# MoayedHajiAli/ElasticDiffusion-official

Hardware: AMD Instinct MI355X
Metric: images/sec at 50 steps (SDXL 2048x1024) (higher is better)
Workload: dtype fp16

## Files before the change

elasticdiffusion_official_amd/csrc/attention_kernels.hip:

```cpp
#include <hip/hip_runtime.h>
#include <stdint.h>

#include "elastic_hip.h"

namespace {

constexpr int D = 64;
constexpr int QB = 128;
constexpr int KT = 64;
constexpr int K_LD = 72;
constexpr int V_LD_TR = 96;
constexpr int V_LD_T = 68;

typedef float f32x16 __attribute__((ext_vector_type(16)));
typedef float f32x8 __attribute__((ext_vector_type(8)));
typedef short s16x4 __attribute__((ext_vector_type(4)));
typedef short s16x8 __attribute__((ext_vector_type(8)));
typedef __bf16 bf16x8 __attribute__((ext_vector_type(8)));
typedef _Float16 f16x8 __attribute__((ext_vector_type(8)));

struct alignas(16) Vec16 { uint32_t w[4]; };
struct alignas(8) Vec8 { uint32_t w[2]; };

struct BF {
  typedef bf16x8 v8;
  static __device__ __forceinline__ f32x16 mfma(v8 a, v8 b, f32x16 c) {
    return __builtin_amdgcn_mfma_f32_32x32x16_bf16(a, b, c, 0, 0, 0);
  }
  static __device__ __forceinline__ v8 pack(f32x8 p) { return __builtin_convertvector(p, v8); }
};
struct HF {
  typedef f16x8 v8;
  static __device__ __forceinline__ f32x16 mfma(v8 a, v8 b, f32x16 c) {
    return __builtin_amdgcn_mfma_f32_32x32x16_f16(a, b, c, 0, 0, 0);
  }
  static __device__ __forceinline__ v8 pack(f32x8 p) { return __builtin_convertvector(p, v8); }
};

template <typename V8>
__device__ __forceinline__ V8 as_v8(Vec16 x) {
  return __builtin_bit_cast(V8, x);
}

struct Params {
  const uint16_t* q;
  const uint16_t* k;
  const uint16_t* v;
  uint16_t* o;
  int Nq, Nk, H, BH, nqb;
  int64_t q_sb, q_sn, k_sb, k_sn, v_sb, v_sn, o_sb, o_sn;
  float scale_log2e;
};

template <bool TR>
// ... 174 lines not shown
          const int row = 16 * st + 4 * hi + ((lane & 15) >> 2);
          const int col = 32 * db + 16 * ((lane >> 4) & 1) + 4 * (lane & 3);
          typedef s16x4 __attribute__((address_space(3))) * lds_s16x4_ptr;
          const s16x4 lo = __builtin_amdgcn_ds_read_tr16_b64_v4i16((lds_s16x4_ptr)(&sm.v[buf][row * V_LD_TR + col]));
          const s16x4 hi4 = __builtin_amdgcn_ds_read_tr16_b64_v4i16((lds_s16x4_ptr)(&sm.v[buf][(row + 8) * V_LD_TR + col]));
          const s16x8 both = __builtin_shufflevector(lo, hi4, 0, 1, 2, 3, 4, 5, 6, 7);
          vf = __builtin_bit_cast(Vec16, both);
        } else {
          const uint16_t* vrow = &sm.v[buf][(32 * db + ln) * V_LD_T + 16 * st + 4 * hi];
          const Vec8 lo = *reinterpret_cast<const Vec8*>(vrow);
          const Vec8 hi8 = *reinterpret_cast<const Vec8*>(vrow + 8);
          vf.w[0] = lo.w[0], vf.w[1] = lo.w[1], vf.w[2] = hi8.w[0], vf.w[3] = hi8.w[1];
        }
#pragma unroll
        for (int qn = 0; qn < QN; ++qn) oacc[qn][db] = T::mfma(as_v8<typename T::v8>(vf), pf[qn], oacc[qn][db]);
      }
    }

    if (t + 1 < n_tiles) write_lds(buf ^ 1);
    __syncthreads();
  }

#pragma unroll
  for (int qn = 0; qn < QN; ++qn) {
    const float l_tot = l_run[qn] + __shfl_xor(l_run[qn], 32, 64);
    const float inv = 1.0f / l_tot;
    if (q_row[qn] < p.Nq) {
      uint16_t* orow = og + (int64_t)q_row[qn] * p.o_sn;
#pragma unroll
      for (int db = 0; db < 2; ++db)
#pragma unroll
        for (int g = 0; g < 4; ++g) {
          f32x8 tmp;
#pragma unroll
          for (int e = 0; e < 4; ++e) tmp[e] = oacc[qn][db][4 * g + e] * inv, tmp[4 + e] = 0.f;
          const Vec16 packed = __builtin_bit_cast(Vec16, T::pack(tmp));
          Vec8 out8 = {{packed.w[0], packed.w[1]}};
          *reinterpret_cast<Vec8*>(orow + 32 * db + 8 * g + 4 * hi) = out8;
        }
    }
  }
}


constexpr float RESCALE_LOG2 = 6.0f;
constexpr float RESCALE_SUM_MAX = 64.0f;

template <int NK>
struct SmemPipe {
  uint16_t k[NK][KT * K_LD];
  uint16_t v[3][KT * V_LD_TR];
};

template <typename T>
__device__ __forceinline__ void qk_tile(const uint16_t* kt, int ln, int hi, const typename T::v8 (&qf)[4], f32x16 (&s)[2]) {
#pragma unroll
  for (int i = 0; i < 16; ++i) s[0][i] = s[1][i] = 0.f;
#pragma unroll
  for (int ks = 0; ks < 4; ++ks)
#pragma unroll
    for (int kb = 0; kb < 2; ++kb) {
      const Vec16 kf = *reinterpret_cast<const Vec16*>(&kt[(32 * kb + ln) * K_LD + 16 * ks + 8 * hi]);
      s[kb] = T::mfma(as_v8<typename T::v8>(kf), qf[ks], s[kb]);
    }
}

__device__ __forceinline__ Vec16 v_frag_tr(const uint16_t* vt, int lane, int hi, int st, int db) {
  const int row = 16 * st + 4 * hi + ((lane & 15) >> 2);
  const int col = 32 * db + 16 * ((lane >> 4) & 1) + 4 * (lane & 3);
  typedef s16x4 __attribute__((address_space(3))) * lds_s16x4_ptr;
  const s16x4 lo = __builtin_amdgcn_ds_read_tr16_b64_v4i16((lds_s16x4_ptr)(&vt[row * V_LD_TR + col]));
  const s16x4 hi4 = __builtin_amdgcn_ds_read_tr16_b64_v4i16((lds_s16x4_ptr)(&vt[(row + 8) * V_LD_TR + col]));
  return __builtin_bit_cast(Vec16, __builtin_shufflevector(lo, hi4, 0, 1, 2, 3, 4, 5, 6, 7));
}

template <typename T>
__device__ __forceinline__ void pv_tile(const uint16_t* vt, int lane, int hi, const typename T::v8 (&pf)[4], f32x16 (&o)[2]) {
#pragma unroll
  for (int st = 0; st < 4; ++st)
#pragma unroll
    for (int db = 0; db < 2; ++db)
      o[db] = T::mfma(as_v8<typename T::v8>(v_frag_tr(vt, lane, hi, st, db)), pf[st], o[db]);
}

typedef __amdgpu_buffer_rsrc_t BufRsrc;
typedef uint32_t u32x4 __attribute__((ext_vector_type(4)));
__device__ __forceinline__ BufRsrc make_rsrc(const void* base, int64_t bytes) {
  const uint64_t a = (uint64_t)base;
  const uint32_t lo = __builtin_amdgcn_readfirstlane((int)(uint32_t)a), hi = __builtin_amdgcn_readfirstlane((int)(uint32_t)(a >> 32));
  const uint32_t n = __builtin_amdgcn_readfirstlane((int)(uint32_t)(bytes > 0xffffffffll ? 0xffffffffll : (bytes < 0 ? 0 : bytes)));
  return __builtin_amdgcn_make_buffer_rsrc((void*)(((uint64_t)hi << 32) | lo),  0, (int)n, 0x00020000);
}
__device__ __forceinline__ Vec16 buf_load16(BufRsrc rs, uint32_t voff, uint32_t soff) {
  const u32x4 v = __builtin_bit_cast(u32x4, __builtin_amdgcn_raw_buffer_load_b128(rs, voff, soff, 0));
  Vec16 o = {{v[0], v[1], v[2], v[3]}};
  return o;
}


template <typename T, int NDB = 2>
__device__ __forceinline__ void store_o_row(uint16_t* orow, const f32x16 (&o)[NDB], float inv, int hi, bool valid, int dh = 64) {
#pragma unroll
  for (int db = 0; db < NDB; ++db) {
    uint32_t part[4][2];
#pragma unroll
    for (int g = 0; g < 4; ++g) {
      f32x8 tmp;
#pragma unroll
      for (int e = 0; e < 4; ++e) tmp[e] = o[db][4 * g + e] * inv, tmp[4 + e] = 0.f;
      const Vec16 packed = __builtin_bit_cast(Vec16, T::pack(tmp));
      part[g][0] = packed.w[0], part[g][1] = packed.w[1];
    }
#pragma unroll
    for (int gp = 0; gp < 2; ++gp) {
      const int ge = 2 * gp, go = 2 * gp + 1;
      const uint32_t r0 = __shfl_xor(hi ? part[ge][0] : part[go][0], 32, 64);
      const uint32_t r1 = __shfl_xor(hi ? part[ge][1] : part[go][1], 32, 64);
      Vec16 out;
      if (hi) out = Vec16{{r0, r1, part[go][0], part[go][1]}};
      else out = Vec16{{part[ge][0], part[ge][1], r0, r1}};
      const int d0 = 32 * db + 8 * (hi ? go : ge);
      if (valid && d0 < dh) *reinterpret_cast<Vec16*>(orow + d0) = out;
    }
  }
}

struct True { static constexpr bool value = true; };
struct False { static constexpr bool value = false; };

struct SoftmaxRun {
  float mb;
  float l;
  float mx;
  float use;
  float alpha;
  float psum;
};

template <typename T>
__device__ __forceinline__ void softmax_slice(int i, f32x16 (&s)[2], float sl, SoftmaxRun& r, typename T::v8 (&pf)[4]) {
  if (i < 2) {
    float mx = (i == 0) ? -INFINITY : r.mx;
#pragma unroll
    for (int j = 0; j < 16; j += 2) mx = fmaxf(fmaxf(mx, s[i][j]), s[i][j + 1]);
    r.mx = mx;
    asm volatile("" : "+v"(r.mx));
  } else if (i == 2) {
    const float mx = fmaxf(r.mx, __shfl_xor(r.mx, 32, 64));
    const float mbn = mx * sl;
    r.use = (mbn - r.mb > RESCALE_LOG2) ? mbn : r.mb;
    r.alpha = __builtin_amdgcn_exp2f(r.mb - r.use);
    r.mb = r.use;
    r.psum = 0.f;
    asm volatile("" : "+v"(r.use), "+v"(r.alpha));
  } else if (i < 15) {
    const int g = (i - 3) / 3, w = (i - 3) % 3;
    const int f0 = 8 * g + 3 * w, n = (w == 2) ? 2 : 3;
#pragma unroll
    for (int j = 0; j < n; ++j) {
      const int f = f0 + j;
      const float e = __builtin_amdgcn_exp2f(__builtin_fmaf(s[f >> 4][f & 15], sl, -r.use));
      s[f >> 4][f & 15] = e;
      r.psum += e;
    }
    asm volatile("" : "+v"(r.psum));
    if (w == 2) {
      f32x8 pv;
#pragma unroll
      for (int j = 0; j < 8; ++j) pv[j] = s[g >> 1][8 * (g & 1) + j];
      pf[g] = T::pack(pv);
      asm volatile("" : "+v"(pf[g]));
    }
  } else {
    r.l = __builtin_fmaf(r.l, r.alpha, r.psum);
  }
}

template <typename T, bool EXP2>
__device__ __forceinline__ void softmax_slice_lazy(int i, f32x16 (&s)[2], float sl, SoftmaxRun& r, typename T::v8 (&pf)[4]) {
  if (i == 0) r.psum = 0.f;
#pragma unroll
  for (int j = 0; j < 2; ++j) {
    const int f = 2 * i + j;
    const float e = EXP2 ? __builtin_amdgcn_exp2f(s[f >> 4][f & 15])
                         : __builtin_amdgcn_exp2f(__builtin_fmaf(s[f >> 4][f & 15], sl, -r.mb));
    s[f >> 4][f & 15] = e;
    r.psum += e;
  }
  asm volatile("" : "+v"(r.psum));
  if ((i & 3) == 3) {
    const int g = i >> 2;
    f32x8 pv;
#pragma unroll
    for (int j = 0; j < 8; ++j) pv[j] = s[g >> 1][8 * (g & 1) + j];
    pf[g] = T::pack(pv);
    asm volatile("" : "+v"(pf[g]));
  }
}

template <typename T>
__device__ __forceinline__ void resoftmax_tile(const uint16_t* kt, int ln, int hi, const typename T::v8 (&qf)[4],
                                               f32x16 (&s)[2], float sl, SoftmaxRun& r, typename T::v8 (&pf)[4]) {
  qk_tile<T>(kt, ln, hi, qf, s);
  float mx = s[0][0];
#pragma unroll
  for (int j = 1; j < 16; ++j) mx = fmaxf(mx, s[0][j]);
#pragma unroll
  for (int j = 0; j < 16; ++j) mx = fmaxf(mx, s[1][j]);
  mx = fmaxf(mx, __shfl_xor(mx, 32, 64));
  const float use = fmaxf(r.mb, mx * sl);
  r.alpha = __builtin_amdgcn_exp2f(r.mb - use);
  r.mb = use;
  float psum = 0.f;
#pragma unroll
  for (int g = 0; g < 4; ++g) {
    f32x8 pv;
#pragma unroll
    for (int j = 0; j < 8; ++j) {
      const int f = 8 * g + j;
      pv[j] = __builtin_amdgcn_exp2f(__builtin_fmaf(s[f >> 4][f & 15], sl, -use));
      psum += pv[j];
    }
    pf[g] = T::pack(pv);
  }
  r.psum = psum;
}

template <typename T, bool HAS_PV, bool HAS_NEXT, bool LAZY, bool EXP2, int DEPTH, class Filler>
__device__ __forceinline__ void pipe_region(Filler&& filler, const uint16_t* k_next, const uint16_t* v_prev, int lane, int ln, int hi,
                                            const typename T::v8 (&qf)[4], f32x16 (&s_cur)[2], f32x16 (&s_next)[2],
                                            const typename T::v8 (&p_prev)[4], typename T::v8 (&p_cur)[4],
                                            f32x16 (&o)[2], float sl, SoftmaxRun& run, const f32x16& negm) {
  constexpr int NQK = HAS_NEXT ? 8 : 0, N = NQK + (HAS_PV ? 8 : 0);
  auto fetch = [&](int i) -> Vec16 {
    if (i < NQK) return *reinterpret_cast<const Vec16*>(&k_next[(32 * (i & 1) + ln) * K_LD + 16 * (i >> 1) + 8 * hi]);
    const int j = i - NQK;
    return v_frag_tr(v_prev, lane, hi, j >> 1, j & 1);
  };
  if (HAS_NEXT && !EXP2) {
#pragma unroll
    for (int i = 0; i < 16; ++i) s_next[0][i] = s_next[1][i] = 0.f;
  }
  Vec16 ring[DEPTH + 1];
#pragma unroll
  for (int r = 0; r <= DEPTH; ++r) ring[r] = Vec16{{0u, 0u, 0u, 0u}};
#pragma unroll
  for (int r = 0; r < DEPTH; ++r)
    if (r < N) ring[r] = fetch(r);
#pragma unroll
  for (int i = 0; i < 16; ++i) {
    if (i < N) {
      if (i + DEPTH < N) ring[(i + DEPTH) % (DEPTH + 1)] = fetch(i + DEPTH);
      const Vec16 a_cur = ring[i % (DEPTH + 1)];
      if (i < NQK) {
        if (EXP2 && i < 2) s_next[i & 1] = T::mfma(as_v8<typename T::v8>(a_cur), qf[0], negm);
        else s_next[i & 1] = T::mfma(as_v8<typename T::v8>(a_cur), qf[i >> 1], s_next[i & 1]);
        asm volatile("" : "+v"(s_next[i & 1]));
      } else {
        const int j = i - NQK;
        o[j & 1] = T::mfma(as_v8<typename T::v8>(a_cur), p_prev[j >> 1], o[j & 1]);
        asm volatile("" : "+v"(o[j & 1]));
      }
    }
    if (LAZY) softmax_slice_lazy<T, EXP2>(i, s_cur, sl, run, p_cur);
    else softmax_slice<T>(i, s_cur, sl, run, p_cur);
    filler(i);
    __builtin_amdgcn_sched_barrier(0);
  }
}

template <typename T, bool LAZY, bool EXP2 = false, int DEPTH = 1, int WAVES = 4>
__global__ void __launch_bounds__(64 * WAVES, 2)
k_flash_attn_pipe(const Params p) {
  static_assert(LAZY || !EXP2, "the exponent-domain variant is built on the lazy-maximum loop");
  static_assert(WAVES == 4 || WAVES == 8, "4 or 8 waves per workgroup");
  constexpr int NK = LAZY ? 3 : 2;
  constexpr int NST = 8 / WAVES;
  __shared__ SmemPipe<NK> sm;
  const int tid = threadIdx.x;
  const int lane = tid & 63, wave = tid >> 6;
  const int ln = lane & 31, hi = lane >> 5;
  int bh, qblk;
  {
    const int id = blockIdx.x, per = 8 * p.nqb, grp = id / per, r = id - grp * per;
    if ((grp + 1) * 8 <= p.BH) {
      bh = grp * 8 + (r & 7);
      qblk = r >> 3;
    } else {
      bh = grp * 8 + r / p.nqb;
      qblk = r % p.nqb;
    }
  }
  const int b = bh / p.H, h = bh - b * p.H;
  const uint16_t* qg = p.q + b * p.q_sb + h * D;
  const uint16_t* kg = p.k + b * p.k_sb + h * D;
  const uint16_t* vg = p.v + b * p.v_sb + h * D;
  uint16_t* og = p.o + b * p.o_sb + h * D;

  const int q_row = qblk * (32 * WAVES) + wave * 32 + ln;
  typename T::v8 qf[4];
#pragma unroll
  for (int ks = 0; ks < 4; ++ks) qf[ks] = as_v8<typename T::v8>(load_row16(qg, p.q_sn, q_row, p.Nq, 16 * ks + 8 * hi));

  const BufRsrc k_rs = make_rsrc(kg, ((int64_t)(p.Nk - 1) * p.k_sn + D) * 2);
  const BufRsrc v_rs = make_rsrc(vg, ((int64_t)(p.Nk - 1) * p.v_sn + D) * 2);
  const int st_row = tid >> 3, st_col = (tid & 7) * 8;
  const uint32_t k_off = (uint32_t)(((int64_t)st_row * p.k_sn + st_col) * 2), k_half = (uint32_t)(32 * p.k_sn * 2);
  const uint32_t v_off = (uint32_t)(((int64_t)st_row * p.v_sn + st_col) * 2), v_half = (uint32_t)(32 * p.v_sn * 2);
  Vec16 kreg[NST], vreg[NST];
  auto load_k = [&](int t) {
    const uint32_t base = k_off + (uint32_t)t * 2u * k_half;
#pragma unroll
    for (int i = 0; i < NST; ++i) kreg[i] = buf_load16(k_rs, base + i * k_half, 0);
  };
  auto load_v = [&](int t) {
    const uint32_t base = v_off + (uint32_t)t * 2u * v_half;
#pragma unroll
    for (int i = 0; i < NST; ++i) vreg[i] = buf_load16(v_rs, base + i * v_half, 0);
  };
  auto write_k = [&](int buf) {
#pragma unroll
    for (int i = 0; i < NST; ++i) *reinterpret_cast<Vec16*>(&sm.k[buf][(st_row + 32 * i) * K_LD + st_col]) = kreg[i];
  };
  auto write_v = [&](int buf) {
#pragma unroll
    for (int i = 0; i < NST; ++i) *reinterpret_cast<Vec16*>(&sm.v[buf][(st_row + 32 * i) * V_LD_TR + st_col]) = vreg[i];
  };

  f32x16 oacc[2];
#pragma unroll
  for (int i = 0; i < 16; ++i) oacc[0][i] = oacc[1][i] = 0.f;
  SoftmaxRun run;
  run.mb = -INFINITY, run.l = 0.f, run.mx = 0.f, run.use = 0.f, run.alpha = 1.f, run.psum = 0.f;
  const float sl = EXP2 ? 1.0f : p.scale_log2e;
  const int n_tiles = (p.Nk + KT - 1) / KT, n_full = p.Nk / KT;
  f32x16 negm;
#pragma unroll
  for (int i = 0; i < 16; ++i) negm[i] = 0.f;

  load_k(0);
  load_v(0);
  Vec16 k1reg[NST];
#pragma unroll
  for (int i = 0; i < NST; ++i) k1reg[i] = buf_load16(k_rs, k_off + 2u * k_half + i * k_half, 0);
  write_k(0);
  write_v(0);
#pragma unroll
  for (int i = 0; i < NST; ++i) *reinterpret_cast<Vec16*>(&sm.k[1][(st_row + 32 * i) * K_LD + st_col]) = k1reg[i];
  __syncthreads();

  f32x16 sA[2], sB[2];
  typename T::v8 pA[4], pB[4];
  int vb_prev = 2, vb_cur = 0, vb_next = 1;
  int kb_cur = 0, kb_next = 1, kb_write = NK == 3 ? 2 : 0;

  auto iter = [&](auto has_pv, auto has_next, int t, f32x16 (&s_cur)[2], f32x16 (&s_next)[2],
                  typename T::v8 (&p_prev)[4], typename T::v8 (&p_cur)[4]) {
    const uint32_t kbase = k_off + (uint32_t)(t + 2) * 2u * k_half, vbase = v_off + (uint32_t)(t + 1) * 2u * v_half;
    uint16_t* const kdst = sm.k[kb_write];
    uint16_t* const vdst = sm.v[vb_next];
    auto filler = [&](int i) {
      if (i < NST) kreg[i] = buf_load16(k_rs, kbase + i * k_half, 0);
      else if (i < 2 * NST) vreg[i - NST] = buf_load16(v_rs, vbase + (i - NST) * v_half, 0);
      else if (i >= 11 && i < 11 + NST) *reinterpret_cast<Vec16*>(&kdst[(st_row + 32 * (i - 11)) * K_LD + st_col]) = kreg[i - 11];
      else if (i >= 11 + NST && i < 11 + 2 * NST)
        *reinterpret_cast<Vec16*>(&vdst[(st_row + 32 * (i - 11 - NST)) * V_LD_TR + st_col]) = vreg[i - 11 - NST];
    };
    constexpr bool lazy = LAZY && (EXP2 || decltype(has_pv)::value);
    pipe_region<T, decltype(has_pv)::value, decltype(has_next)::value, lazy, EXP2, DEPTH>(filler, sm.k[kb_next], sm.v[vb_prev], lane, ln,
                                                                                          hi, qf, s_cur, s_next, p_prev, p_cur,
                                                                                          oacc, sl, run, negm);
    if (lazy) {
      run.alpha = 1.0f;
      if (__any(!(run.psum <= RESCALE_SUM_MAX))) {
        const float mb_old = run.mb;
        resoftmax_tile<T>(sm.k[kb_cur], ln, hi, qf, s_cur, sl, run, p_cur);
        if (EXP2) {
          const float d = run.mb - mb_old;
          if (decltype(has_next)::value) {
#pragma unroll
            for (int i = 0; i < 16; ++i) s_next[0][i] -= d, s_next[1][i] -= d;
          }
#pragma unroll
          for (int i = 0; i < 16; ++i) negm[i] = -run.mb;
          asm volatile("" : "+v"(negm));
        }
      }
      run.l = __builtin_fmaf(run.l, run.alpha, run.psum);
    }
    if (__any(run.alpha != 1.0f)) {
#pragma unroll
      for (int i = 0; i < 16; ++i) {
        oacc[0][i] *= run.alpha;
        oacc[1][i] *= run.alpha;
      }
    }
    const int tmp = vb_prev;
    vb_prev = vb_cur, vb_cur = vb_next, vb_next = tmp;
    const int ktmp = kb_cur;
    kb_cur = kb_next, kb_next = kb_write, kb_write = NK == 3 ? ktmp : kb_cur;
    __syncthreads();
  };

  if (n_full > 0) {
    qk_tile<T>(sm.k[0], ln, hi, qf, sA);
    if (EXP2) {
      float mx = sA[0][0];
#pragma unroll
      for (int j = 1; j < 16; ++j) mx = fmaxf(mx, sA[0][j]);
#pragma unroll
      for (int j = 0; j < 16; ++j) mx = fmaxf(mx, sA[1][j]);
      mx = fmaxf(mx, __shfl_xor(mx, 32, 64));
      run.mb = mx;
#pragma unroll
      for (int i = 0; i < 16; ++i) sA[0][i] -= mx, sA[1][i] -= mx, negm[i] = -mx;
      asm volatile("" : "+v"(negm));
    }
    __syncthreads();
    if (n_full == 1) {
      iter(False{}, False{}, 0, sA, sB, pB, pA);
    } else {
      iter(False{}, True{}, 0, sA, sB, pB, pA);
      int t = 1;
      for (; t + 2 < n_full; t += 2) {
        iter(True{}, True{}, t, sB, sA, pA, pB);
        iter(True{}, True{}, t + 1, sA, sB, pB, pA);
      }
      if (n_full - t == 2) {
        iter(True{}, True{}, t, sB, sA, pA, pB);
        iter(True{}, False{}, t + 1, sA, sB, pB, pA);
      } else {
        iter(True{}, False{}, t, sB, sA, pA, pB);
      }
    }
    if ((n_full - 1) & 1) pv_tile<T>(sm.v[vb_prev], lane, hi, pB, oacc);
    else pv_tile<T>(sm.v[vb_prev], lane, hi, pA, oacc);
  }

  if (n_tiles > n_full) {
    f32x16 s[2];
    qk_tile<T>(sm.k[kb_cur], ln, hi, qf, s);
#pragma unroll
    for (int kb = 0; kb < 2; ++kb)
#pragma unroll
      for (int r = 0; r < 16; ++r)
        if (n_full * KT + 32 * kb + 8 * (r >> 2) + 4 * hi + (r & 3) >= p.Nk) s[kb][r] = -INFINITY;
    float mx = s[0][0];
#pragma unroll
    for (int r = 1; r < 16; ++r) mx = fmaxf(mx, s[0][r]);
#pragma unroll
    for (int r = 0; r < 16; ++r) mx = fmaxf(mx, s[1][r]);
    mx = fmaxf(mx, __shfl_xor(mx, 32, 64));
    const float use = fmaxf(run.mb, mx * sl);
    const float alpha = __builtin_amdgcn_exp2f(run.mb - use);
    float psum = 0.f;
#pragma unroll
    for (int kb = 0; kb < 2; ++kb)
#pragma unroll
      for (int r = 0; r < 16; ++r) {
        const float e = __builtin_amdgcn_exp2f(__builtin_fmaf(s[kb][r], sl, -use));
        s[kb][r] = e;
        psum += e;
      }
    run.l = __builtin_fmaf(run.l, alpha, psum);
#pragma unroll
    for (int i = 0; i < 16; ++i) {
      oacc[0][i] *= alpha;
      oacc[1][i] *= alpha;
    }
    typename T::v8 pf[4];
#pragma unroll
    for (int st = 0; st < 4; ++st) {
      f32x8 pv;
#pragma unroll
      for (int j = 0; j < 8; ++j) pv[j] = s[st >> 1][8 * (st & 1) + j];
      pf[st] = T::pack(pv);
    }
    pv_tile<T>(sm.v[vb_cur], lane, hi, pf, oacc);
  }

  const float l_tot = run.l + __shfl_xor(run.l, 32, 64);
  const float inv = 1.0f / l_tot;
  store_o_row<T>(og + (int64_t)q_row * p.o_sn, oacc, inv, hi, q_row < p.Nq);
}

constexpr int SK_QBLOCKS = 4;

template <int NKB>
struct SmemSmall {
  uint16_t k[32 * NKB * K_LD];
  uint16_t v[32 * NKB * V_LD_TR];
};

template <typename T, int NKB>
__global__ void __launch_bounds__(256, 2)
k_flash_attn_smallkv(const Params p) {
  __shared__ SmemSmall<NKB> sm;
  const int tid = threadIdx.x;
  const int lane = tid & 63, wave = tid >> 6;
  const int ln = lane & 31, hi = lane >> 5;
  const int nqg = p.nqb;
  const int bh = blockIdx.x / nqg, qgrp = blockIdx.x - bh * nqg;
  const int b = bh / p.H, h = bh - b * p.H;
  const uint16_t* qg = p.q + b * p.q_sb + h * D;
  const uint16_t* kg = p.k + b * p.k_sb + h * D;
  const uint16_t* vg = p.v + b * p.v_sb + h * D;
  uint16_t* og = p.o + b * p.o_sb + h * D;

  for (int idx = tid; idx < 32 * NKB * 8; idx += 256) {
    const int row = idx >> 3, col = (idx & 7) * 8;
    *reinterpret_cast<Vec16*>(&sm.k[row * K_LD + col]) = load_row16(kg, p.k_sn, row, p.Nk, col);
    *reinterpret_cast<Vec16*>(&sm.v[row * V_LD_TR + col]) = load_row16(vg, p.v_sn, row, p.Nk, col);
  }
  __syncthreads();
  const float sl = p.scale_log2e;

  for (int qb = 0; qb < SK_QBLOCKS; ++qb) {
    const int q_row = (qgrp * SK_QBLOCKS + qb) * QB + wave * 32 + ln;
    if ((qgrp * SK_QBLOCKS + qb) * QB + wave * 32 >= p.Nq) break;
    typename T::v8 qf[4];
#pragma unroll
    for (int ks = 0; ks < 4; ++ks) qf[ks] = as_v8<typename T::v8>(load_row16(qg, p.q_sn, q_row, p.Nq, 16 * ks + 8 * hi));
    f32x16 s[NKB];
#pragma unroll
    for (int kb = 0; kb < NKB; ++kb)
#pragma unroll
      for (int i = 0; i < 16; ++i) s[kb][i] = 0.f;
#pragma unroll
    for (int ks = 0; ks < 4; ++ks)
#pragma unroll
      for (int kb = 0; kb < NKB; ++kb) {
// ... 469 lines not shown
        const int row = 16 * st + 4 * hi + ((lane & 15) >> 2);
        const int col = 32 * db + 16 * ((lane >> 4) & 1) + 4 * (lane & 3);
        typedef s16x4 __attribute__((address_space(3))) * lds_s16x4_ptr;
        const s16x4 lo = __builtin_amdgcn_ds_read_tr16_b64_v4i16((lds_s16x4_ptr)(&sm.v[buf][row * G::VLD + col]));
        const s16x4 hi4 = __builtin_amdgcn_ds_read_tr16_b64_v4i16((lds_s16x4_ptr)(&sm.v[buf][(row + 8) * G::VLD + col]));
        const Vec16 vf = __builtin_bit_cast(Vec16, __builtin_shufflevector(lo, hi4, 0, 1, 2, 3, 4, 5, 6, 7));
        oacc[db] = T::mfma(as_v8<typename T::v8>(vf), pf, oacc[db]);
      }
    }
    if (t + 1 < n_tiles) write_lds(buf ^ 1);
    __syncthreads();
  }

  const float l_tot = l_run + __shfl_xor(l_run, 32, 64);
  const float inv = 1.0f / l_tot;
  store_o_row<T, G::NDB>(og + (int64_t)q_row * p.o_sn, oacc, inv, hi, q_row < p.Nq, DH);
}

}

extern "C" {

int ed_flash_attention(const void* q, const void* k, const void* v, void* out, int dtype, int B, int H, int Nq, int Nk,
                       int head_dim, int64_t q_sb, int64_t q_sn, int64_t k_sb, int64_t k_sn, int64_t v_sb, int64_t v_sn,
                       int64_t o_sb, int64_t o_sn, float scale, int v_path, void* stream) {
  if (B == 0 || H == 0 || Nq == 0) return 0;
  if (Nk <= 0) return (int)hipErrorInvalidValue;
  if (head_dim != D) {
    if (head_dim != 40 && head_dim != 80 && head_dim != 160) return (int)hipErrorInvalidValue;
    if (dtype != ED_BF16 && dtype != ED_F16) return (int)hipErrorInvalidValue;
    if ((((uintptr_t)q | (uintptr_t)k | (uintptr_t)v) & 15u) || ((uintptr_t)out & 7u)) return (int)hipErrorInvalidValue;
    if ((q_sb | q_sn | k_sb | k_sn | v_sb | v_sn) % 8 || (o_sb | o_sn) % 4) return (int)hipErrorInvalidValue;
    Params p;
    p.q = (const uint16_t*)q, p.k = (const uint16_t*)k, p.v = (const uint16_t*)v, p.o = (uint16_t*)out;
    p.Nq = Nq, p.Nk = Nk, p.H = H, p.BH = B * H, p.nqb = (Nq + QB - 1) / QB;
    p.q_sb = q_sb, p.q_sn = q_sn, p.k_sb = k_sb, p.k_sn = k_sn, p.v_sb = v_sb, p.v_sn = v_sn, p.o_sb = o_sb, p.o_sn = o_sn;
    p.scale_log2e = scale * 1.44269504088896340736f;
    const int64_t nb = (int64_t)p.BH * p.nqb;
    if (nb > 0x7fffffff) return (int)hipErrorInvalidValue;
    const dim3 grid((unsigned)nb), block(256);
    hipStream_t st = (hipStream_t)stream;
#define ED_FG(DHV)                                                                      \
  if (dtype == ED_BF16) k_flash_attn_gen<BF, DHV><<<grid, block, 0, st>>>(p);           \
  else k_flash_attn_gen<HF, DHV><<<grid, block, 0, st>>>(p);
    if (head_dim == 40) { ED_FG(40) } else if (head_dim == 80) { ED_FG(80) } else { ED_FG(160) }
#undef ED_FG
    return (int)hipGetLastError();
  }
  if ((((uintptr_t)q | (uintptr_t)k | (uintptr_t)v) & 15u) || ((uintptr_t)out & 7u)) return (int)hipErrorInvalidValue;
  if ((q_sb | q_sn | k_sb | k_sn | v_sb | v_sn) % 8 || (o_sb | o_sn) % 4) return (int)hipErrorInvalidValue;
  Params p;
  p.q = (const uint16_t*)q, p.k = (const uint16_t*)k, p.v = (const uint16_t*)v, p.o = (uint16_t*)out;
  hipStream_t st = (hipStream_t)stream;
  if ((v_path >= 4 && v_path <= 10)) {
    if (v_path == 8 && Nk > 160) return (int)hipErrorInvalidValue;
    if ((v_path == 6 || v_path == 7 || v_path == 9 || v_path == 10) && Nk < 64) return (int)hipErrorInvalidValue;
    if (v_path != 8 && ((int64_t)(Nk + 2 * KT) * (k_sn > v_sn ? k_sn : v_sn) * 2 >= 0x7fffffffll)) return (int)hipErrorInvalidValue;
    const int rows_per_wg = v_path == 8 ? QB * SK_QBLOCKS : (v_path >= 9 ? 2 * QB : QB);
    p.Nq = Nq, p.Nk = Nk, p.H = H, p.BH = B * H, p.nqb = (Nq + rows_per_wg - 1) / rows_per_wg;
    p.q_sb = q_sb, p.q_sn = q_sn, p.k_sb = k_sb, p.k_sn = k_sn, p.v_sb = v_sb, p.v_sn = v_sn, p.o_sb = o_sb, p.o_sn = o_sn;
    p.scale_log2e = scale * 1.44269504088896340736f;
    const int64_t nb = (int64_t)p.BH * p.nqb;
    if (nb > 0x7fffffff) return (int)hipErrorInvalidValue;
    const dim3 grid((unsigned)nb), block(256);
    if (dtype != ED_BF16 && dtype != ED_F16) return (int)hipErrorInvalidValue;
    if (v_path == 4) {
      if (dtype == ED_BF16) k_flash_attn_pipe<BF, false><<<grid, block, 0, st>>>(p);
      else k_flash_attn_pipe<HF, false><<<grid, block, 0, st>>>(p);
    } else if (v_path == 5) {
      if (dtype == ED_BF16) k_flash_attn_pipe<BF, true><<<grid, block, 0, st>>>(p);
      else k_flash_attn_pipe<HF, true><<<grid, block, 0, st>>>(p);
    } else if (v_path == 6) {
      if (dtype == ED_BF16) k_flash_attn_pipe<BF, true, true><<<grid, block, 0, st>>>(p);
      else k_flash_attn_pipe<HF, true, true><<<grid, block, 0, st>>>(p);
    } else if (v_path == 7) {
      if (dtype == ED_BF16) k_flash_attn_pipe<BF, false, false, 3><<<grid, block, 0, st>>>(p);
      else k_flash_attn_pipe<HF, false, false, 3><<<grid, block, 0, st>>>(p);
    } else if (v_path == 9) {
      if (dtype == ED_BF16) k_flash_attn_pipe<BF, false, false, 1, 8><<<grid, dim3(512), 0, st>>>(p);
      else k_flash_attn_pipe<HF, false, false, 1, 8><<<grid, dim3(512), 0, st>>>(p);
    } else if (v_path == 10) {
      if (dtype == ED_BF16) k_flash_attn_pipe<BF, true, false, 1, 8><<<grid, dim3(512), 0, st>>>(p);
      else k_flash_attn_pipe<HF, true, false, 1, 8><<<grid, dim3(512), 0, st>>>(p);
    } else if (Nk <= 64) {
      if (dtype == ED_BF16) k_flash_attn_smallkv<BF, 2><<<grid, block, 0, st>>>(p);
      else k_flash_attn_smallkv<HF, 2><<<grid, block, 0, st>>>(p);
    } else if (Nk <= 96) {
      if (dtype == ED_BF16) k_flash_attn_smallkv<BF, 3><<<grid, block, 0, st>>>(p);
      else k_flash_attn_smallkv<HF, 3><<<grid, block, 0, st>>>(p);
    } else {
      if (dtype == ED_BF16) k_flash_attn_smallkv<BF, 5><<<grid, block, 0, st>>>(p);
      else k_flash_attn_smallkv<HF, 5><<<grid, block, 0, st>>>(p);
    }
    return (int)hipGetLastError();
  }
  const int qn = (v_path & 2) ? 2 : 1;
  p.Nq = Nq, p.Nk = Nk, p.H = H, p.BH = B * H, p.nqb = (Nq + QB * qn - 1) / (QB * qn);
  p.q_sb = q_sb, p.q_sn = q_sn, p.k_sb = k_sb, p.k_sn = k_sn, p.v_sb = v_sb, p.v_sn = v_sn, p.o_sb = o_sb, p.o_sn = o_sn;
  p.scale_log2e = scale * 1.44269504088896340736f;
  const int64_t blocks = (int64_t)p.BH * p.nqb;
  if (blocks > 0x7fffffff) return (int)hipErrorInvalidValue;
  const dim3 grid((unsigned)blocks), block(256);
#define ED_FA(T)                                                                 \
  if (v_path == 0) k_flash_attn_fwd<T, true, 1><<<grid, block, 0, st>>>(p);      \
  else if (v_path == 1) k_flash_attn_fwd<T, false, 1><<<grid, block, 0, st>>>(p); \
  else if (v_path == 2) k_flash_attn_fwd<T, true, 2><<<grid, block, 0, st>>>(p);  \
  else if (v_path == 3) k_flash_attn_fwd<T, false, 2><<<grid, block, 0, st>>>(p); \
  else return (int)hipErrorInvalidValue;
  if (dtype == ED_BF16) {
    ED_FA(BF)
  } else if (dtype == ED_F16) {
    ED_FA(HF)
  } else {
    return (int)hipErrorInvalidValue;
  }
#undef ED_FA
  return (int)hipGetLastError();
}

int ed_flash_attention_ip(const void* q, const void* k, const void* v, void* out, int dtype, int B, int H, int Nq, int Nt, int Ni,
                          int head_dim, int64_t q_sb, int64_t q_sn, int64_t k_sb, int64_t k_sn, int64_t v_sb, int64_t v_sn,
                          int64_t o_sb, int64_t o_sn, float scale, float ip_scale, void* stream) {
  if (head_dim != D || Nt < 1 || Nt > 160 || Ni < 1 || Ni > 32) return (int)hipErrorInvalidValue;
  if (dtype != ED_BF16 && dtype != ED_F16) return (int)hipErrorInvalidValue;
  if (B < 0 || H < 0 || Nq < 0) return (int)hipErrorInvalidValue;
  if (B == 0 || H == 0 || Nq == 0) return 0;
  if ((((uintptr_t)q | (uintptr_t)k | (uintptr_t)v) & 15u) || ((uintptr_t)out & 7u)) return (int)hipErrorInvalidValue;
  if ((q_sb | q_sn | k_sb | k_sn | v_sb | v_sn) % 8 || (o_sb | o_sn) % 4) return (int)hipErrorInvalidValue;
  ParamsIp pi;
  Params& p = pi.p;
  p.q = (const uint16_t*)q, p.k = (const uint16_t*)k, p.v = (const uint16_t*)v, p.o = (uint16_t*)out;
  p.Nq = Nq, p.Nk = Nt, p.H = H, p.BH = B * H, p.nqb = (Nq + QB * SK_QBLOCKS - 1) / (QB * SK_QBLOCKS);
  p.q_sb = q_sb, p.q_sn = q_sn, p.k_sb = k_sb, p.k_sn = k_sn, p.v_sb = v_sb, p.v_sn = v_sn, p.o_sb = o_sb, p.o_sn = o_sn;
  p.scale_log2e = scale * 1.44269504088896340736f;
  pi.Ni = Ni, pi.ip_scale = ip_scale;
  const int64_t nb = (int64_t)p.BH * p.nqb;
// ... 49 lines not shown
```

elasticdiffusion_official_amd/ops.py:

```python
import ctypes
import math

import torch

from . import _hip

ED_F32, ED_F16, ED_BF16 = 0, 1, 2
_DTYPE = {torch.float32: ED_F32, torch.float16: ED_F16, torch.bfloat16: ED_BF16}


_LAUNCH = {"device": None}


def _stream_of(t):
    if _LAUNCH["device"] is None:
        _LAUNCH["device"] = t.device
    return _stream()


def _stream():
    dev = _LAUNCH["device"]
    if dev is None:
        raise RuntimeError("internal: _stream() before any device tensor argument")
    return torch.cuda.current_stream(dev).cuda_stream
# ... 1204 lines not shown


VAE_ATTENTION_CHUNK_BYTES = 1 << 30


def vae_attention(q, k, v, key_bias=None):
    B, N, C = q.shape
    scale = C ** -0.5
    rows = max(64, min(N, VAE_ATTENTION_CHUNK_BYTES // (4 * N * B) // 64 * 64)) if N > 256 else N
    kt = k.transpose(1, 2)
    if rows >= N:
        return torch.bmm(softmax_rows_(torch.bmm(q, kt), scale, key_bias), v)
    out = torch.empty_like(q)
    for a in range(0, N, rows):
        s = torch.bmm(q[:, a:a + rows], kt)
        out[:, a:a + rows] = torch.bmm(softmax_rows_(s, scale, key_bias), v)
    return out


FLASH_V_PATH = None
FLASH_HEAD_DIMS = (40, 64, 80, 160)
FLASH_EXP2 = False
_ENV_VARIANT = __import__("os").environ.get("ED_FLASH_VARIANT")
LOG2E = 1.4426950408889634


def _pipe_fits(Nk, row_stride):
    return Nk >= 128 and (Nk + 128) * row_stride * 2 < 2 ** 31


def flash_prescale(Nq, Nk, row_stride, scale=0.125):
    if FLASH_V_PATH is not None:
        want = int(FLASH_V_PATH)
    elif _ENV_VARIANT is not None:
        want = -1 if _ENV_VARIANT == "legacy" else int(_ENV_VARIANT)
    else:
        want = 6 if FLASH_EXP2 else -1
    return scale * LOG2E if (want == 6 and _pipe_fits(Nk, row_stride)) else None


def _flash_variant(B, heads, Nq, Nk, k=None, v=None, prescaled=False):
    fits = k is None or _pipe_fits(Nk, max(k.stride(1), v.stride(1)))
    if prescaled:
        if not (Nk >= 128 and fits):
            _reject("flash_attention: exponent-domain q needs the pipelined kernel (Nk >= 128, 32-bit K / V offsets)")
        return 6
    if FLASH_V_PATH is not None and int(FLASH_V_PATH) != 6:
        return int(FLASH_V_PATH)
    legacy = 2 if (Nq >= 2048 and Nk >= 1024 and B * heads * (Nq // 256) >= 1024) else 0
    if _ENV_VARIANT == "legacy":
        return legacy
    if _ENV_VARIANT is not None and int(_ENV_VARIANT) != 6:
        want = int(_ENV_VARIANT)
        if want in (4, 5, 7, 9, 10):
            return want if (Nk >= 128 and fits) else (8 if Nk <= 96 else legacy)
        return want if (want != 8 or Nk <= SMALLKV_MAX_KEYS) else legacy
    if Nk <= 96 or _stream_two_chunks(Nq, Nk):
        return 8
    if Nk >= 128 and fits:
        return FLASH_DEFAULT_PIPE
    return legacy


SMALLKV_MAX_KEYS = 160


def _stream_two_chunks(Nq, Nk):
    return 128 <= Nk <= SMALLKV_MAX_KEYS and Nq >= 4096


FLASH_DEFAULT_PIPE = 5


def flash_attention(q, k, v, heads, v_path=None, prescaled=False):
    B, Nq, HD = q.shape
    Nk = k.shape[1]
    hd = HD // heads
    if HD != heads * hd or hd not in FLASH_HEAD_DIMS or k.shape != (B, Nk, HD) or v.shape != (B, Nk, HD):
        _reject(f"flash_attention: head_dim must be one of {FLASH_HEAD_DIMS} and shapes consistent (q {tuple(q.shape)}, "
                f"k {tuple(k.shape)}, v {tuple(v.shape)}, heads {heads})")
    if hd != 64 and (prescaled or v_path is not None):
        _reject("flash_attention: kernel variants exist for head_dim 64 only")
    for t, name in ((q, "q"), (k, "k"), (v, "v")):
        if not t.is_cuda or t.dtype != q.dtype or t.stride(2) != 1:
            _reject(f"flash_attention: {name} must be a 16-bit tensor on the MI355X with unit last stride; no CPU fallback")
        if _LAUNCH["device"] is None:
            _LAUNCH["device"] = t.device
        elif _LAUNCH["device"] != t.device:
            _reject(f"flash_attention: {name} lives on {t.device}, q on {_LAUNCH['device']}")
    if v_path is not None and (int(v_path) == 6) != bool(prescaled):
        _reject("flash_attention: v_path 6 takes exponent-domain q (prescaled=True) and nothing else does")
    out = torch.empty(B, Nq, HD, dtype=q.dtype, device=q.device)
    TIMER.note_work("ed_flash_attention", flops=4.0 * B * heads * Nq * Nk * hd,
                    nbytes=2.0 * q.element_size() * HD * B * (Nq + Nk))
    variant = 0 if hd != 64 else (_flash_variant(B, heads, Nq, Nk, k, v, prescaled) if v_path is None else int(v_path))
    _call("ed_flash_attention", q.data_ptr(), k.data_ptr(), v.data_ptr(), out.data_ptr(), _code(q, "q"), B, heads, Nq, Nk,
          hd, q.stride(0), q.stride(1), k.stride(0), k.stride(1), v.stride(0), v.stride(1), out.stride(0), out.stride(1),
          hd ** -0.5, variant, _stream())
    return out


IP_MAX_TEXT_KEYS = SMALLKV_MAX_KEYS
IP_MAX_IMAGE_KEYS = 32


def flash_attention_ip_ok(head_dim, n_text, n_image):
    return head_dim == 64 and 1 <= n_text <= IP_MAX_TEXT_KEYS and 1 <= n_image <= IP_MAX_IMAGE_KEYS


def flash_attention_ip(q, k, v, heads, n_text, ip_scale):
    B, Nq, HD = q.shape
    N = k.shape[1]
    hd = HD // heads
    n_text, ip_scale = int(n_text), float(ip_scale)
    if HD != heads * hd or hd != 64 or k.shape != (B, N, HD) or v.shape != (B, N, HD):
        _reject(f"flash_attention_ip: head_dim must be 64 and shapes consistent (q {tuple(q.shape)}, k {tuple(k.shape)}, "
                f"v {tuple(v.shape)}, heads {heads})")
    if not flash_attention_ip_ok(hd, n_text, N - n_text):
        _reject(f"flash_attention_ip: needs 1 <= text keys <= {IP_MAX_TEXT_KEYS} and 1 <= image keys <= {IP_MAX_IMAGE_KEYS}, "
                f"got {n_text} and {N - n_text}")
    if ip_scale != ip_scale or ip_scale in (float("inf"), float("-inf")):
# ... 606 lines not shown
```

Baseline: 0.1064.

## Add LDS-DMA flash attention variant with swizzled K/V tiles for selected shapes

Adds a pipelined flash-attention variant that streams K and V tiles from global memory directly into LDS using buffer_load ... lds, instead of loading into registers and then writing to shared memory. LDS tiles are unpadded and XOR-swizzled to avoid bank conflicts, and the fragment reads are adjusted to match. The variant is picked by default only for a small set of self-attention shapes. It cuts register staging and VGPR pressure, but adds a full vmcnt wait before each barrier, which may reduce load/compute overlap.

```diff
diff --git a/elasticdiffusion_official_amd/csrc/attention_kernels.hip b/elasticdiffusion_official_amd/csrc/attention_kernels.hip
--- a/elasticdiffusion_official_amd/csrc/attention_kernels.hip
+++ b/elasticdiffusion_official_amd/csrc/attention_kernels.hip
@@ -1,5 +1,7 @@
 #include <hip/hip_runtime.h>
 #include <stdint.h>
+
+#include <type_traits>
 
 #include "elastic_hip.h"
 
@@ -280,7 +282,18 @@
   uint16_t v[3][KT * V_LD_TR];
 };
 
-template <typename T>
+struct alignas(1024) SmemPipeDma {
+  uint16_t k[3][KT * D];
+  uint16_t v[3][KT * D];
+};
+
+template <bool SWZ>
+__device__ __forceinline__ int k_frag_off(int ln, int hi, int kb, int ks) {
+  if (SWZ) return (32 * kb + ln) * D + 8 * ((2 * ks + hi) ^ ((ln >> 1) & 7));
+  return (32 * kb + ln) * K_LD + 16 * ks + 8 * hi;
+}
+
+template <typename T, bool SWZ = false>
 __device__ __forceinline__ void qk_tile(const uint16_t* kt, int ln, int hi, const typename T::v8 (&qf)[4], f32x16 (&s)[2]) {
 #pragma unroll
   for (int i = 0; i < 16; ++i) s[0][i] = s[1][i] = 0.f;
@@ -288,27 +301,30 @@
   for (int ks = 0; ks < 4; ++ks)
 #pragma unroll
     for (int kb = 0; kb < 2; ++kb) {
-      const Vec16 kf = *reinterpret_cast<const Vec16*>(&kt[(32 * kb + ln) * K_LD + 16 * ks + 8 * hi]);
+      const Vec16 kf = *reinterpret_cast<const Vec16*>(&kt[k_frag_off<SWZ>(ln, hi, kb, ks)]);
       s[kb] = T::mfma(as_v8<typename T::v8>(kf), qf[ks], s[kb]);
     }
 }
 
+template <bool SWZ = false>
 __device__ __forceinline__ Vec16 v_frag_tr(const uint16_t* vt, int lane, int hi, int st, int db) {
+  constexpr int LD = SWZ ? D : V_LD_TR;
   const int row = 16 * st + 4 * hi + ((lane & 15) >> 2);
-  const int col = 32 * db + 16 * ((lane >> 4) & 1) + 4 * (lane & 3);
+  int col = 32 * db + 16 * ((lane >> 4) & 1) + 4 * (lane & 3);
+  if (SWZ) col ^= 32 * ((lane >> 3) & 1);
   typedef s16x4 __attribute__((address_space(3))) * lds_s16x4_ptr;
-  const s16x4 lo = __builtin_amdgcn_ds_read_tr16_b64_v4i16((lds_s16x4_ptr)(&vt[row * V_LD_TR + col]));
-  const s16x4 hi4 = __builtin_amdgcn_ds_read_tr16_b64_v4i16((lds_s16x4_ptr)(&vt[(row + 8) * V_LD_TR + col]));
+  const s16x4 lo = __builtin_amdgcn_ds_read_tr16_b64_v4i16((lds_s16x4_ptr)(&vt[row * LD + col]));
+  const s16x4 hi4 = __builtin_amdgcn_ds_read_tr16_b64_v4i16((lds_s16x4_ptr)(&vt[(row + 8) * LD + col]));
   return __builtin_bit_cast(Vec16, __builtin_shufflevector(lo, hi4, 0, 1, 2, 3, 4, 5, 6, 7));
 }
 
-template <typename T>
+template <typename T, bool SWZ = false>
 __device__ __forceinline__ void pv_tile(const uint16_t* vt, int lane, int hi, const typename T::v8 (&pf)[4], f32x16 (&o)[2]) {
 #pragma unroll
   for (int st = 0; st < 4; ++st)
 #pragma unroll
     for (int db = 0; db < 2; ++db)
-      o[db] = T::mfma(as_v8<typename T::v8>(v_frag_tr(vt, lane, hi, st, db)), pf[st], o[db]);
+      o[db] = T::mfma(as_v8<typename T::v8>(v_frag_tr<SWZ>(vt, lane, hi, st, db)), pf[st], o[db]);
 }
 
 typedef __amdgpu_buffer_rsrc_t BufRsrc;
@@ -324,6 +340,23 @@
   Vec16 o = {{v[0], v[1], v[2], v[3]}};
   return o;
 }
+typedef __attribute__((address_space(3))) uint16_t* lds_u16_ptr;
+__device__ __forceinline__ u32x4 make_rsrc_words(const void* base, int64_t bytes) {
+  const uint64_t a = (uint64_t)base;
+  u32x4 r;
+  r[0] = __builtin_amdgcn_readfirstlane((int)(uint32_t)a);
+  r[1] = __builtin_amdgcn_readfirstlane((int)((uint32_t)(a >> 32) & 0xffffu));
+  r[2] = __builtin_amdgcn_readfirstlane((int)(uint32_t)(bytes > 0xffffffffll ? 0xffffffffll : (bytes < 0 ? 0 : bytes)));
+  r[3] = 0x00020000u;
+  return r;
+}
+#pragma clang diagnostic push
+#pragma clang diagnostic ignored "-Winline-asm"
+__device__ __forceinline__ void buf_load16_lds(u32x4 rs, uint16_t* dst, uint32_t voff) {
+  const uint32_t lds_addr = (uint32_t)(uintptr_t)(lds_u16_ptr)dst;
+  asm volatile("s_mov_b32 m0, %0\n\ts_nop 0\n\tbuffer_load_dwordx4 %1, %2, 0 offen lds" : : "s"(lds_addr), "v"(voff), "s"(rs) : "memory", "m0");
+}
+#pragma clang diagnostic pop
 
 
 template <typename T, int NDB = 2>
@@ -426,10 +459,10 @@
   }
 }
 
-template <typename T>
+template <typename T, bool SWZ = false>
 __device__ __forceinline__ void resoftmax_tile(const uint16_t* kt, int ln, int hi, const typename T::v8 (&qf)[4],
                                                f32x16 (&s)[2], float sl, SoftmaxRun& r, typename T::v8 (&pf)[4]) {
-  qk_tile<T>(kt, ln, hi, qf, s);
+  qk_tile<T, SWZ>(kt, ln, hi, qf, s);
   float mx = s[0][0];
 #pragma unroll
   for (int j = 1; j < 16; ++j) mx = fmaxf(mx, s[0][j]);
@@ -454,16 +487,19 @@
   r.psum = psum;
 }
 
-template <typename T, bool HAS_PV, bool HAS_NEXT, bool LAZY, bool EXP2, int DEPTH, class Filler>
+template <typename T, bool HAS_PV, bool HAS_NEXT, bool LAZY, bool EXP2, int DEPTH, bool SWZ, class Filler>
 __device__ __forceinline__ void pipe_region(Filler&& filler, const uint16_t* k_next, const uint16_t* v_prev, int lane, int ln, int hi,
                                             const typename T::v8 (&qf)[4], f32x16 (&s_cur)[2], f32x16 (&s_next)[2],
                                             const typename T::v8 (&p_prev)[4], typename T::v8 (&p_cur)[4],
                                             f32x16 (&o)[2], float sl, SoftmaxRun& run, const f32x16& negm) {
   constexpr int NQK = HAS_NEXT ? 8 : 0, N = NQK + (HAS_PV ? 8 : 0);
   auto fetch = [&](int i) -> Vec16 {
-    if (i < NQK) return *reinterpret_cast<const Vec16*>(&k_next[(32 * (i & 1) + ln) * K_LD + 16 * (i >> 1) + 8 * hi]);
+    if (i < NQK) {
+      if constexpr (SWZ) return *reinterpret_cast<const Vec16*>(&k_next[k_frag_off<true>(ln, hi, i & 1, i >> 1)]);
+      else return *reinterpret_cast<const Vec16*>(&k_next[(32 * (i & 1) + ln) * K_LD + 16 * (i >> 1) + 8 * hi]);
+    }
     const int j = i - NQK;
-    return v_frag_tr(v_prev, lane, hi, j >> 1, j & 1);
+    return v_frag_tr<SWZ>(v_prev, lane, hi, j >> 1, j & 1);
   };
   if (HAS_NEXT && !EXP2) {
 #pragma unroll
@@ -497,14 +533,15 @@
   }
 }
 
-template <typename T, bool LAZY, bool EXP2 = false, int DEPTH = 1, int WAVES = 4>
+template <typename T, bool LAZY, bool EXP2 = false, int DEPTH = 1, int WAVES = 4, bool DMA = false>
 __global__ void __launch_bounds__(64 * WAVES, 2)
 k_flash_attn_pipe(const Params p) {
   static_assert(LAZY || !EXP2, "the exponent-domain variant is built on the lazy-maximum loop");
   static_assert(WAVES == 4 || WAVES == 8, "4 or 8 waves per workgroup");
+  static_assert(!DMA || LAZY, "the LDS-DMA image is a ring of three K buffers");
   constexpr int NK = LAZY ? 3 : 2;
   constexpr int NST = 8 / WAVES;
-  __shared__ SmemPipe<NK> sm;
+  __shared__ typename std::conditional<DMA, SmemPipeDma, SmemPipe<NK>>::type sm;
   const int tid = threadIdx.x;
   const int lane = tid & 63, wave = tid >> 6;
   const int ln = lane & 31, hi = lane >> 5;
@@ -533,8 +570,13 @@
   const BufRsrc k_rs = make_rsrc(kg, ((int64_t)(p.Nk - 1) * p.k_sn + D) * 2);
   const BufRsrc v_rs = make_rsrc(vg, ((int64_t)(p.Nk - 1) * p.v_sn + D) * 2);
   const int st_row = tid >> 3, st_col = (tid & 7) * 8;
-  const uint32_t k_off = (uint32_t)(((int64_t)st_row * p.k_sn + st_col) * 2), k_half = (uint32_t)(32 * p.k_sn * 2);
-  const uint32_t v_off = (uint32_t)(((int64_t)st_row * p.v_sn + st_col) * 2), v_half = (uint32_t)(32 * p.v_sn * 2);
+  const int k_col = DMA ? ((tid & 7) ^ ((st_row >> 1) & 7)) * 8 : st_col;
+  const int v_col = DMA ? ((tid & 7) ^ (((st_row >> 1) & 1) << 2)) * 8 : st_col;
+  const uint32_t k_off = (uint32_t)(((int64_t)st_row * p.k_sn + k_col) * 2), k_half = (uint32_t)(32 * p.k_sn * 2);
+  const uint32_t v_off = (uint32_t)(((int64_t)st_row * p.v_sn + v_col) * 2), v_half = (uint32_t)(32 * p.v_sn * 2);
+  const u32x4 k_rw = DMA ? make_rsrc_words(kg, ((int64_t)(p.Nk - 1) * p.k_sn + D) * 2) : u32x4{};
+  const u32x4 v_rw = DMA ? make_rsrc_words(vg, ((int64_t)(p.Nk - 1) * p.v_sn + D) * 2) : u32x4{};
+  const int dma_row = DMA ? 8 * __builtin_amdgcn_readfirstlane(wave) : 0;
   Vec16 kreg[NST], vreg[NST];
   auto load_k = [&](int t) {
     const uint32_t base = k_off + (uint32_t)t * 2u * k_half;
@@ -554,6 +596,8 @@
 #pragma unroll
     for (int i = 0; i < NST; ++i) *reinterpret_cast<Vec16*>(&sm.v[buf][(st_row + 32 * i) * V_LD_TR + st_col]) = vreg[i];
   };
+  auto dma_k = [&](uint16_t* dst, int t, int i) { buf_load16_lds(k_rw, dst + (dma_row + 32 * i) * D, k_off + (uint32_t)t * 2u * k_half + i * k_half); };
+  auto dma_v = [&](uint16_t* dst, int t, int i) { buf_load16_lds(v_rw, dst + (dma_row + 32 * i) * D, v_off + (uint32_t)t * 2u * v_half + i * v_half); };
 
   f32x16 oacc[2];
 #pragma unroll
@@ -566,15 +610,25 @@
 #pragma unroll
   for (int i = 0; i < 16; ++i) negm[i] = 0.f;
 
-  load_k(0);
-  load_v(0);
-  Vec16 k1reg[NST];
-#pragma unroll
-  for (int i = 0; i < NST; ++i) k1reg[i] = buf_load16(k_rs, k_off + 2u * k_half + i * k_half, 0);
-  write_k(0);
-  write_v(0);
-#pragma unroll
-  for (int i = 0; i < NST; ++i) *reinterpret_cast<Vec16*>(&sm.k[1][(st_row + 32 * i) * K_LD + st_col]) = k1reg[i];
+  if constexpr (DMA) {
+#pragma unroll
+    for (int i = 0; i < NST; ++i) dma_k(sm.k[0], 0, i);
+#pragma unroll
+    for (int i = 0; i < NST; ++i) dma_v(sm.v[0], 0, i);
+#pragma unroll
+    for (int i = 0; i < NST; ++i) dma_k(sm.k[1], 1, i);
+    asm volatile("s_waitcnt vmcnt(0)" ::: "memory");
+  } else {
+    load_k(0);
+    load_v(0);
+    Vec16 k1reg[NST];
+#pragma unroll
+    for (int i = 0; i < NST; ++i) k1reg[i] = buf_load16(k_rs, k_off + 2u * k_half + i * k_half, 0);
+    write_k(0);
+    write_v(0);
+#pragma unroll
+    for (int i = 0; i < NST; ++i) *reinterpret_cast<Vec16*>(&sm.k[1][(st_row + 32 * i) * K_LD + st_col]) = k1reg[i];
+  }
   __syncthreads();
 
   f32x16 sA[2], sB[2];
@@ -588,6 +642,11 @@
     uint16_t* const kdst = sm.k[kb_write];
     uint16_t* const vdst = sm.v[vb_next];
     auto filler = [&](int i) {
+      if (DMA) {
+        if (i < NST) dma_k(kdst, t + 2, i);
+        else if (i < 2 * NST) dma_v(vdst, t + 1, i - NST);
+        return;
+      }
       if (i < NST) kreg[i] = buf_load16(k_rs, kbase + i * k_half, 0);
       else if (i < 2 * NST) vreg[i - NST] = buf_load16(v_rs, vbase + (i - NST) * v_half, 0);
       else if (i >= 11 && i < 11 + NST) *reinterpret_cast<Vec16*>(&kdst[(st_row + 32 * (i - 11)) * K_LD + st_col]) = kreg[i - 11];
@@ -595,14 +654,14 @@
         *reinterpret_cast<Vec16*>(&vdst[(st_row + 32 * (i - 11 - NST)) * V_LD_TR + st_col]) = vreg[i - 11 - NST];
     };
     constexpr bool lazy = LAZY && (EXP2 || decltype(has_pv)::value);
-    pipe_region<T, decltype(has_pv)::value, decltype(has_next)::value, lazy, EXP2, DEPTH>(filler, sm.k[kb_next], sm.v[vb_prev], lane, ln,
+    pipe_region<T, decltype(has_pv)::value, decltype(has_next)::value, lazy, EXP2, DEPTH, DMA>(filler, sm.k[kb_next], sm.v[vb_prev], lane, ln,
                                                                                           hi, qf, s_cur, s_next, p_prev, p_cur,
                                                                                           oacc, sl, run, negm);
     if (lazy) {
       run.alpha = 1.0f;
       if (__any(!(run.psum <= RESCALE_SUM_MAX))) {
         const float mb_old = run.mb;
-        resoftmax_tile<T>(sm.k[kb_cur], ln, hi, qf, s_cur, sl, run, p_cur);
+        resoftmax_tile<T, DMA>(sm.k[kb_cur], ln, hi, qf, s_cur, sl, run, p_cur);
         if (EXP2) {
           const float d = run.mb - mb_old;
           if (decltype(has_next)::value) {
@@ -627,11 +686,12 @@
     vb_prev = vb_cur, vb_cur = vb_next, vb_next = tmp;
     const int ktmp = kb_cur;
     kb_cur = kb_next, kb_next = kb_write, kb_write = NK == 3 ? ktmp : kb_cur;
+    if (DMA) asm volatile("s_waitcnt vmcnt(0)" ::: "memory");
     __syncthreads();
   };
 
   if (n_full > 0) {
-    qk_tile<T>(sm.k[0], ln, hi, qf, sA);
+    qk_tile<T, DMA>(sm.k[0], ln, hi, qf, sA);
     if (EXP2) {
       float mx = sA[0][0];
 #pragma unroll
@@ -661,13 +721,13 @@
         iter(True{}, False{}, t, sB, sA, pA, pB);
       }
     }
-    if ((n_full - 1) & 1) pv_tile<T>(sm.v[vb_prev], lane, hi, pB, oacc);
-    else pv_tile<T>(sm.v[vb_prev], lane, hi, pA, oacc);
+    if ((n_full - 1) & 1) pv_tile<T, DMA>(sm.v[vb_prev], lane, hi, pB, oacc);
+    else pv_tile<T, DMA>(sm.v[vb_prev], lane, hi, pA, oacc);
   }
 
   if (n_tiles > n_full) {
     f32x16 s[2];
-    qk_tile<T>(sm.k[kb_cur], ln, hi, qf, s);
+    qk_tile<T, DMA>(sm.k[kb_cur], ln, hi, qf, s);
 #pragma unroll
     for (int kb = 0; kb < 2; ++kb)
 #pragma unroll
@@ -704,7 +764,7 @@
       for (int j = 0; j < 8; ++j) pv[j] = s[st >> 1][8 * (st & 1) + j];
       pf[st] = T::pack(pv);
     }
-    pv_tile<T>(sm.v[vb_cur], lane, hi, pf, oacc);
+    pv_tile<T, DMA>(sm.v[vb_cur], lane, hi, pf, oacc);
   }
 
   const float l_tot = run.l + __shfl_xor(run.l, 32, 64);
@@ -1280,11 +1340,11 @@
   Params p;
   p.q = (const uint16_t*)q, p.k = (const uint16_t*)k, p.v = (const uint16_t*)v, p.o = (uint16_t*)out;
   hipStream_t st = (hipStream_t)stream;
-  if ((v_path >= 4 && v_path <= 10)) {
+  if ((v_path >= 4 && v_path <= 11)) {
     if (v_path == 8 && Nk > 160) return (int)hipErrorInvalidValue;
-    if ((v_path == 6 || v_path == 7 || v_path == 9 || v_path == 10) && Nk < 64) return (int)hipErrorInvalidValue;
+    if ((v_path == 6 || v_path == 7 || v_path >= 9) && Nk < 64) return (int)hipErrorInvalidValue;
     if (v_path != 8 && ((int64_t)(Nk + 2 * KT) * (k_sn > v_sn ? k_sn : v_sn) * 2 >= 0x7fffffffll)) return (int)hipErrorInvalidValue;
-    const int rows_per_wg = v_path == 8 ? QB * SK_QBLOCKS : (v_path >= 9 ? 2 * QB : QB);
+    const int rows_per_wg = v_path == 8 ? QB * SK_QBLOCKS : (v_path == 9 || v_path == 10 ? 2 * QB : QB);
     p.Nq = Nq, p.Nk = Nk, p.H = H, p.BH = B * H, p.nqb = (Nq + rows_per_wg - 1) / rows_per_wg;
     p.q_sb = q_sb, p.q_sn = q_sn, p.k_sb = k_sb, p.k_sn = k_sn, p.v_sb = v_sb, p.v_sn = v_sn, p.o_sb = o_sb, p.o_sn = o_sn;
     p.scale_log2e = scale * 1.44269504088896340736f;
@@ -1310,6 +1370,9 @@
     } else if (v_path == 10) {
       if (dtype == ED_BF16) k_flash_attn_pipe<BF, true, false, 1, 8><<<grid, dim3(512), 0, st>>>(p);
       else k_flash_attn_pipe<HF, true, false, 1, 8><<<grid, dim3(512), 0, st>>>(p);
+    } else if (v_path == 11) {
+      if (dtype == ED_BF16) k_flash_attn_pipe<BF, true, false, 1, 4, true><<<grid, block, 0, st>>>(p);
+      else k_flash_attn_pipe<HF, true, false, 1, 4, true><<<grid, block, 0, st>>>(p);
     } else if (Nk <= 64) {
       if (dtype == ED_BF16) k_flash_attn_smallkv<BF, 2><<<grid, block, 0, st>>>(p);
       else k_flash_attn_smallkv<HF, 2><<<grid, block, 0, st>>>(p);
diff --git a/elasticdiffusion_official_amd/ops.py b/elasticdiffusion_official_amd/ops.py
--- a/elasticdiffusion_official_amd/ops.py
+++ b/elasticdiffusion_official_amd/ops.py
@@ -1280,13 +1280,13 @@
         return legacy
     if _ENV_VARIANT is not None and int(_ENV_VARIANT) != 6:
         want = int(_ENV_VARIANT)
-        if want in (4, 5, 7, 9, 10):
+        if want in (4, 5, 7, 9, 10, 11):
             return want if (Nk >= 128 and fits) else (8 if Nk <= 96 else legacy)
         return want if (want != 8 or Nk <= SMALLKV_MAX_KEYS) else legacy
     if Nk <= 96 or _stream_two_chunks(Nq, Nk):
         return 8
     if Nk >= 128 and fits:
-        return FLASH_DEFAULT_PIPE
+        return 11 if (FLASH_DEFAULT_PIPE == 5 and _lds_dma_gains(B, heads, Nq, Nk)) else FLASH_DEFAULT_PIPE
     return legacy
 
 
@@ -1295,6 +1295,13 @@
 
 def _stream_two_chunks(Nq, Nk):
     return 128 <= Nk <= SMALLKV_MAX_KEYS and Nq >= 4096
+
+
+FLASH_LDS_DMA_SHAPES = frozenset({(40, 10, 4096), (12, 10, 4096), (40, 20, 1024)})
+
+
+def _lds_dma_gains(B, heads, Nq, Nk):
+    return Nq == Nk and Nk % 64 == 0 and Nk >= 128 and (B, heads, Nk) in FLASH_LDS_DMA_SHAPES
 
 
 FLASH_DEFAULT_PIPE = 5
```

Result: no change. 0.1069, median of 6 (+0.5%).
